# pennneutrinos/chroma

Measured on AMD Instinct MI355X. Metric: photons/sec (propagate_hit), higher is better.
Workload: dtype f32

## Files before the change

chroma_amd/csrc/chroma_hip.hip:

```cpp
#include <math.h>
#include <stdio.h>
#include <stdlib.h>
#include <string.h>
#include <algorithm>

#ifndef CHROMA_EXPERIMENTAL
#define CHROMA_EXPERIMENTAL 0
#endif
#ifndef CHROMA_HYBRID_RENDER
#define CHROMA_HYBRID_RENDER 1
#endif
#include "chroma_internal.h"
#include "propagate_device.h"

#include "kernel_propagate_fused.h"

#include "kernel_step_control.h"

#include "kernels_raycast_crosscheck.h"

#include "kernel_raycast_quad.h"

#include "kernel_raycast_pair.h"

// ... 156 lines not shown
    HIP_TRY(hipMemset(cs.d_counters, 0, sizeof c));
    stats->photon_steps += c.photon_steps;
    stats->nodes_visited += c.nodes_visited;
    stats->triangles_tested += c.triangles_tested;
    stats->stack_overflows += c.stack_overflows;
    stats->stack_spills += c.stack_spills;
    stats->packet_rays += c.packet_rays;
    stats->packet_nodes_visited += c.packet_nodes;
    stats->packet_triangles_tested += c.packet_tris;
    return CHROMA_OK;
}

enum { EV_STEP_BEGIN, EV_PACKET_BEGIN, EV_CAST_BEGIN, EV_CAST_END, EV_PHYSICS_END, EV_STEP_END, EV_PER_STEP };

struct chroma_tracks {
    struct Slab { float4 *rows; uint32_t count; };
    uint64_t nphotons = 0, nrows = 0;
    float4 *rows0 = nullptr;
    uint32_t *offsets = nullptr;
    std::vector<Slab> slabs;
};

static void tracks_release(chroma_ctx *ctx, chroma_tracks *tr)
{
    if (!tr) return;
    for (const chroma_tracks::Slab &s : tr->slabs) chroma_free(ctx, s.rows);
    chroma_free(ctx, tr->rows0);
    chroma_free(ctx, tr->offsets);
    delete tr;
}

namespace { struct PropagateCall; }
static int propagate_order(PropagateCall &call, uint32_t **d_order);

namespace {
struct PropagateCall {
    const CallScope &scope; CallState &cs;
    chroma_ctx *ctx; chroma_geometry *geom;
    CallPlan plan;
    PhotonView pv; chroma_rng rng; chroma_propagate_options opt;
    uint64_t nphotons; uint32_t ncopies;
    uint32_t *in_q, *out_q;
    float4 *work_in, *work_out;
    float4 *rays, *rays_next;
    float4 *final_rec;
    uint32_t final_epoch;
    HitsOut ho;
    bool finalize;
    chroma_propagate_stats acc;
    long long n_upper;
    bool finalized;
    chroma_tracks *tracks;

    hipEvent_t *events(int step) const { return opt.time_kernels ? cs.step_events.data() + EV_PER_STEP * step : nullptr; }

    int load_working()
    {
        const unsigned blocks = (unsigned)std::min<uint64_t>((nphotons + PHYS_BLOCK - 1) / PHYS_BLOCK, (uint64_t)ctx->physics_blocks);
        int rc = scope.clear_words(W_PACKET_USE, W_PACKET_END - W_PACKET_USE); if (rc) return rc;
        uint32_t *d_order = nullptr;
        rc = propagate_order(*this, &d_order); if (rc) return rc;
        hipLaunchKernelGGL(k_load_working, dim3(blocks), dim3(PHYS_BLOCK), 0, ctx->stream, geom->view, pv, in_q, work_in,
                           (uint64_t)nphotons, ncopies, (uint32_t)(nphotons / ncopies), plan.chain ? rays : nullptr,
                           plan.packet == 2 ? cs.d_words + W_PACKET_COHERENT : nullptr, (const uint32_t *)d_order, plan.cast == Cast::LITERAL ? 1 : 0);
        if (d_order) { chroma_free(ctx, d_order); acc.reordered += nphotons; }
#if CHROMA_EXPERIMENTAL
        if (plan.packet)
            hipLaunchKernelGGL(k_packet_decide, dim3(1), dim3(1), 0, ctx->stream, cs.d_words + W_PACKET_COHERENT, cs.d_words + W_PACKET_USE,
                               (uint64_t)nphotons, plan.packet);
#endif
        HIP_TRY(hipGetLastError());
        return CHROMA_OK;
    }

    void launch_step_begin(uint32_t first_n)
    {
        hipLaunchKernelGGL(k_step_begin, dim3(1), dim3(1), 0, ctx->stream, in_q, out_q, cs.d_step,
                           tracks ? 0u : opt.use_weights ? 0xFFFFFFFFu : (uint32_t)(PROP_BLOCK * 16 * 8), first_n);
    }

    void launch_physics(int scatter_first, int fixup)
    {
        StepState *st = cs.d_step;
        float4 *chained = plan.chain ? rays_next : nullptr;
        const bool plain = geom->view.plain_optics != 0;
        bool deal = false;
#if PHYS_DEAL
        deal = plain && !final_rec;
#endif
        const int pb = deal ? PHYS_DEAL_BLOCK : PHYS_BLOCK_OF(!plain);
        unsigned blocks = (unsigned)std::min<long long>((n_upper + pb - 1) / pb, std::max<long long>(1, (long long)ctx->physics_blocks * PHYS_BLOCK / pb));
        if (fixup == 1 && plain) blocks = std::max(std::min(blocks, 64u), blocks / 8);
        DeviceCounters *pc = plan.counting ? cs.d_counters : nullptr;
#if PHYS_DEAL
        if (deal) {
            hipLaunchKernelGGL(k_physics_deal, dim3(blocks), dim3(PHYS_DEAL_BLOCK), 0, ctx->stream, geom->view, pv, st, work_in, out_q, work_out,
                               cs.hit_triangle, cs.hit_distance, rng.seed, rng.photon_id_base, opt.use_weights, scatter_first,
                               cs.retry_list, fixup, pc, chained);
            return;
        }
#endif
        const int literal_rays = fixup == 2 ? 1 : 0;
        with_bool(!plain, [&](auto FULL) {
            hipLaunchKernelGGL((k_physics<FULL>), dim3(blocks), dim3(PHYS_BLOCK_OF(FULL)), 0, ctx->stream, geom->view, pv, st, work_in, out_q,
                               work_out, cs.hit_triangle, cs.hit_distance, rng.seed, rng.photon_id_base, opt.use_weights, scatter_first,
                               cs.retry_list, fixup, pc, chained, final_rec, final_epoch, literal_rays);
        });
    }

    int launch_split_step(int scatter_first, hipEvent_t *ev, uint32_t first_n, bool packet)
    {
        if (n_upper <= 0) return CHROMA_OK;
        StepState *st = cs.d_step;
        const Cast cast = plan.cast;
        const bool exact = cast == Cast::LITERAL || cast == Cast::LITERAL_LANE;
        const dim3 block(PROP_BLOCK);
        auto record = [&](int slot) { return ev ? hipEventRecord(ev[slot], ctx->stream) : hipSuccess; };
        const unsigned rblocks = (unsigned)std::min<long long>((n_upper + PROP_BLOCK - 1) / PROP_BLOCK, 8 * 256);
        auto retry = [&](auto C) {
            hipLaunchKernelGGL((k_raycast_retry<C>), dim3(rblocks), block, 0, ctx->stream, geom->view, rays, st, cs.hit_triangle,
                               cs.hit_distance, cs.retry_list, cs.d_counters);
        };
        launch_step_begin(first_n);
        HIP_TRY(record(EV_STEP_BEGIN));
        if (!plan.chain) {
            unsigned sblocks = (unsigned)std::min<long long>((n_upper + 255) / 256, (long long)ctx->physics_blocks * 4);
            hipLaunchKernelGGL(k_ray_setup, dim3(sblocks), dim3(256), 0, ctx->stream, geom->view, work_in, st, rays,
                               cs.hit_triangle, cs.hit_distance, cs.retry_list, &st->retry, cast == Cast::LITERAL ? 1 : 0);
        }
        HIP_TRY(record(EV_PACKET_BEGIN));
        const uint32_t *skip_quad = nullptr;
#if CHROMA_EXPERIMENTAL
        if (packet) {
            skip_quad = cs.d_words + W_PACKET_USE;
            const unsigned pwaves = (unsigned)std::min<long long>((n_upper + WAVE - 1) / WAVE, (long long)ctx->waves[(int)Cast::QUAD]);
            with_bool(plan.counting, [&](auto C) {
                hipLaunchKernelGGL((k_raycast_packet<C>), dim3(pwaves), block, 0, ctx->stream, geom->view, rays, st, cs.hit_triangle,
                                   cs.hit_distance, cs.retry_list, cs.d_counters, cs.d_words + W_PACKET_USE);
            });
        }
#else
        (void)packet;
#endif
        HIP_TRY(record(EV_CAST_BEGIN));
        const dim3 grid(cast_waves(ctx, cast, n_upper));
        const int chained = plan.chain ? 1 : 0;
        with_bool(plan.counting, [&](auto C) {
            switch (cast) {
            case Cast::PAIR:
                hipLaunchKernelGGL((k_raycast_pair<C>), grid, block, 0, ctx->stream, geom->view, rays, 0, st, cs.hit_triangle,
                                   cs.hit_distance, cs.retry_list, cs.coop_spill, cs.d_counters, ctx->coop_chunk);
                break;
            case Cast::QUAD:
                hipLaunchKernelGGL((k_raycast_quad<C>), grid, block, 0, ctx->stream, geom->view, rays, 0, st, cs.hit_triangle,
                                   cs.hit_distance, cs.retry_list, cs.coop_spill, cs.d_counters, ctx->coop_chunk, chained, skip_quad,
                                   ctx->claim_static);
                break;
            case Cast::COOP:
                hipLaunchKernelGGL((k_raycast_coop<C>), grid, block, 0, ctx->stream, geom->view, rays, 0, st, cs.hit_triangle,
                                   cs.hit_distance, cs.retry_list, cs.coop_spill, cs.d_counters, ctx->coop_chunk);
                break;
            case Cast::WIDE:
                hipLaunchKernelGGL((k_raycast_wide<C>), grid, block, 0, ctx->stream, geom->view, rays, 0, st, cs.hit_triangle,
                                   cs.hit_distance, cs.retry_list, cs.wide_spill, cs.d_counters, ctx->ray_chunk);
                break;
            case Cast::PERSISTENT:
                hipLaunchKernelGGL((k_raycast_persistent<C>), grid, block, 0, ctx->stream, geom->view, rays, 0, st, cs.hit_triangle,
                                   cs.hit_distance, cs.retry_list, cs.d_counters);
                break;
            case Cast::LITERAL:
                hipLaunchKernelGGL((k_raycast_literal<C>), grid, block, 0, ctx->stream, geom->view, rays, st, cs.hit_triangle,
                                   cs.hit_distance, cs.coop_spill, cs.d_counters, ctx->coop_chunk, chained, cs.retry_list,
                                   ctx->claim_static);
                retry(C);
                break;
            case Cast::LITERAL_LANE:
                hipLaunchKernelGGL((k_raycast_retry<C, true>), grid, block, 0, ctx->stream, geom->view, rays, st, cs.hit_triangle,
                                   cs.hit_distance, cs.retry_list, cs.d_counters);
                break;
            }
        });
        HIP_TRY(record(EV_CAST_END));
        launch_physics(scatter_first, exact ? 2 : 0);
        HIP_TRY(record(EV_PHYSICS_END));
        if (!exact) {
            with_bool(plan.counting, retry);
            launch_physics(scatter_first, 1);
        }
        HIP_TRY(record(EV_STEP_END));
        HIP_TRY(hipGetLastError());
        if (plan.chain) std::swap(rays, rays_next);
        return CHROMA_OK;
    }

    int launch_tail(int nsteps, int scatter_first, hipEvent_t *ev, uint32_t first_n, bool *done)
    {
        *done = false;
        const unsigned waves = cast_waves(ctx, Cast::COOP, n_upper);
        if ((long long)waves * 8 < n_upper) return CHROMA_OK;
        launch_step_begin(first_n);
        HitsOut beside; memset(&beside, 0, sizeof beside);
        uint32_t *words = nullptr;
        if (finalize) {
            beside = ho;
            words = cs.d_words;
            int rc = scope.clear_results(); if (rc) return rc;
            if (final_rec)
                hipLaunchKernelGGL(k_mark_tail, dim3(32), dim3(256), 0, ctx->stream, in_q, final_rec, photon_tail_stamp(final_epoch));
            HIP_TRY(hipEventRecord(cs.ev_fork, ctx->stream));
        }
        if (ev) HIP_TRY(hipEventRecord(ev[EV_STEP_BEGIN], ctx->stream));
        with_bool(plan.cast == Cast::LITERAL, [&](auto L) {
            with_bool(plan.counting, [&](auto C) {
                hipLaunchKernelGGL((k_tail_coop<C, L>), dim3(waves), dim3(PROP_BLOCK), 0, ctx->stream, geom->view, pv, cs.d_step, work_in,
                                   rng.seed, rng.photon_id_base, nsteps, opt.use_weights, scatter_first, cs.coop_spill, cs.d_counters, beside, words);
            });
        });
        if (ev) HIP_TRY(hipEventRecord(ev[EV_STEP_END], ctx->stream));
        if (finalize) {
            HIP_TRY(hipStreamWaitEvent(cs.aux_stream, cs.ev_fork, 0));
            launch_finalize(cs.aux_stream, photon_tail_stamp(final_epoch));
            HIP_TRY(hipEventRecord(cs.ev_join, cs.aux_stream));
            HIP_TRY(hipStreamWaitEvent(ctx->stream, cs.ev_join, 0));
            finalized = true;
        }
        HIP_TRY(hipGetLastError());
        *done = true;
        return CHROMA_OK;
    }

    void launch_finalize(hipStream_t stream, uint32_t tail_mark)
    {
        const unsigned blocks = (unsigned)((nphotons + COPY_ITEMS * 256 - 1) / (COPY_ITEMS * 256));
        hipLaunchKernelGGL(k_finalize_hits, dim3(blocks), dim3(256), 0, stream, geom->view, pv, (const float4 *)final_rec, final_epoch,
                           (uint64_t)nphotons, ho, cs.d_words, tail_mark);
    }

    int read_step_times(int steps, int tail_step)
    {
        for (int k = 0; k < steps; k++) {
            const hipEvent_t *ev = events(k);
            float ms = 0.f;
            HIP_TRY(hipEventElapsedTime(&ms, ev[EV_STEP_BEGIN], ev[EV_STEP_END]));
            acc.kernel_ms += ms;
            if (k == tail_step) continue;
            HIP_TRY(hipEventElapsedTime(&ms, ev[EV_CAST_BEGIN], ev[EV_CAST_END]));
            acc.raycast_ms += ms;
            acc.raycast_launches++;
            if (k == 0 && plan.packet) {
                HIP_TRY(hipEventElapsedTime(&ms, ev[EV_PACKET_BEGIN], ev[EV_CAST_BEGIN]));
                acc.packet_ms += ms;
                acc.packet_launches++;
            }
            HIP_TRY(hipEventElapsedTime(&ms, ev[EV_CAST_END], ev[EV_PHYSICS_END]));
            acc.physics_ms += ms;
            acc.physics_launches++;
        }
        return CHROMA_OK;
    }

    int run_device_steps()
    {
        const int max_steps = opt.max_steps;
        HIP_TRY(hipMemsetAsync(cs.d_step, 0, sizeof(StepState), ctx->stream));
        hipLaunchKernelGGL(k_set_word, dim3(1), dim3(1), 0, ctx->stream, in_q, 1u);
        hipLaunchKernelGGL(k_set_word, dim3(1), dim3(1), 0, ctx->stream, out_q, 1u);
        int rc = load_working(); if (rc) return rc;
        const int nev = opt.time_kernels ? EV_PER_STEP * max_steps : 0;
        while ((int)cs.step_events.size() < nev) { hipEvent_t e; HIP_TRY(hipEventCreate(&e)); cs.step_events.push_back(e); }
        const long long few = (long long)PROP_BLOCK * 16 * 8;
        int step = 0, next_check = 1, tail_step = -1;
        bool done = false;
        while (step < max_steps && !done) {
            const int scatter_first = step == 0 ? opt.scatter_first : 0;
            const uint32_t first_n = step == 0 ? (uint32_t)nphotons : 0u;
            if (plan.tail && n_upper < few) {
                rc = launch_tail(max_steps - step, scatter_first, events(step), first_n, &done); if (rc) return rc;
                if (done) { tail_step = step++; break; }
            }
            rc = launch_split_step(scatter_first, events(step), first_n, step == 0 && plan.packet != 0); if (rc) return rc;
            step++;
            std::swap(in_q, out_q);
            std::swap(work_in, work_out);
            if (step == next_check && step < max_steps) {
                rc = scope.read_survivors(in_q, &n_upper); if (rc) return rc;
                if (n_upper <= 0) done = true;
                next_check = (plan.tail_watch && n_upper < 16 * few) ? step + 1 : (step < 8) ? step * 2 : step + 8;
            }
        }
        if (!done) {
            unsigned blocks = (unsigned)std::min<long long>((n_upper + 255) / 256, 4096);
            hipLaunchKernelGGL(k_store_working, dim3(std::max(blocks, 1u)), dim3(256), 0, ctx->stream, geom->view, pv, in_q, work_in);
        }
        HIP_TRY(hipMemcpyAsync(cs.h_step, cs.d_step, sizeof(StepState), hipMemcpyDeviceToHost, ctx->stream));
        HIP_TRY(hipStreamSynchronize(ctx->stream));
        acc.launches += ((const StepState *)cs.h_step)->launches;
        return opt.time_kernels ? read_step_times(step, tail_step) : CHROMA_OK;
    }

    void store_working()
    {
        const unsigned blocks = (unsigned)std::min<long long>((n_upper + 255) / 256, 4096);
        hipLaunchKernelGGL(k_store_working, dim3(std::max(blocks, 1u)), dim3(256), 0, ctx->stream, geom->view, pv, in_q, work_in);
    }

    int run_tracked_steps(uint64_t max_rows)
    {
// ... 83 lines not shown
                HIP_TRY(hipEventElapsedTime(&ms, cs.ev_start, cs.ev_stop));
                acc.kernel_ms += ms;
            }
            step += nsteps;
            scatter_first = 0;
            if (step < max_steps) {
                std::swap(in_q, out_q);
                hipLaunchKernelGGL(k_set_word, dim3(1), dim3(1), 0, ctx->stream, out_q, 1u);
                rc = scope.read_survivors(in_q, &n); if (rc) return rc;
                if (n == 0) break;
            }
        }
        return CHROMA_OK;
    }

    int finish(chroma_hits_request *hr, chroma_propagate_stats *stats, int32_t *aborted)
    {
        int rc = CHROMA_OK;
        if (!finalize) {
            rc = scope.clear_words(W_ABORT); if (rc) return rc;
            const unsigned blocks = (unsigned)std::min<uint64_t>((nphotons + 255) / 256, 4096);
            hipLaunchKernelGGL(k_flags_or, dim3(blocks), dim3(256), 0, ctx->stream, pv.flags, (uint64_t)nphotons, CHROMA_NAN_ABORT,
                               cs.d_words + W_ABORT);
        } else if (!finalized) {
            rc = scope.clear_results(); if (rc) return rc;
            launch_finalize(ctx->stream, 0u);
        }
        HIP_TRY(hipGetLastError());
        rc = scope.read_results(); if (rc) return rc;
        if (hr) hr->nhits = scope.word(W_HIT_COUNT);
        if (aborted) *aborted = (scope.word(W_ABORT) & CHROMA_NAN_ABORT) ? 1 : 0;
        chroma_propagate_stats tmp; memset(&tmp, 0, sizeof tmp);
        chroma_propagate_stats *s = stats ? stats : &tmp;
        rc = stats_read(scope, s); if (rc) return rc;
        if (stats) {
            stats->launches += acc.launches;
            stats->kernel_ms += acc.kernel_ms;
            stats->raycast_ms += acc.raycast_ms;
            stats->raycast_launches += acc.raycast_launches;
            stats->physics_ms += acc.physics_ms;
            stats->physics_launches += acc.physics_launches;
            stats->packet_ms += acc.packet_ms;
            stats->packet_launches += acc.packet_launches;
            stats->reordered += acc.reordered;
        }
        if (s->stack_overflows) return set_error(CHROMA_ERR_STACK, "traversal stack overflowed for %llu rays", (unsigned long long)s->stack_overflows);
        return CHROMA_OK;
    }
};
}

int propagate_settings(const CallScope &scope)
{
    chroma_ctx *ctx = scope.ctx; CallState &cs = scope.state();
    hipDeviceProp_t prop;
    HIP_TRY(hipGetDeviceProperties(&prop, ctx->device));
    ctx->physics_blocks = prop.multiProcessorCount * 8;
    const char *walk = getenv("CHROMA_WALK");
    if (walk) cs.walk = CHROMA_WALK_QUAD;
    for (int w = 0; w < NWALKS; w++) {
        const Walk &row = WALKS[w];
        int per_cu = row.waves_per_cu;
        if (const char *e = getenv(row.waves_env)) per_cu = std::max(1, atoi(e));
        ctx->waves[(int)row.cast] = prop.multiProcessorCount * per_cu;
        if (walk && (!strcmp(walk, row.name) || (row.alias && !strcmp(walk, row.alias)))) cs.walk = w;
    }
#if CHROMA_EXPERIMENTAL
    if (const char *e = getenv("CHROMA_PACKET")) cs.packet_mode = !strcmp(e, "on") ? 1 : !strcmp(e, "auto") ? 2 : 0;
    if (const char *e = getenv("CHROMA_AUTOSORT")) cs.autosort_mode = !strcmp(e, "on") || !strcmp(e, "1") ? 1 : !strcmp(e, "off") || !strcmp(e, "0") ? 0 : 2;
#endif
    if (const char *e = getenv("CHROMA_RAY_CHUNK")) ctx->ray_chunk = std::max(64, atoi(e));
    if (const char *e = getenv("CHROMA_COOP_CHUNK")) ctx->coop_chunk = std::max(8, atoi(e));
    if (const char *e = getenv("CHROMA_CLAIM_STATIC")) { int big = 0, small = 0; if (sscanf(e, "%d:%d", &big, &small) < 2) small = big; ctx->claim_static = std::min(8, std::max(0, big)) | std::min(8, std::max(0, small)) << 4; }
    if (const char *e = getenv("CHROMA_TAIL"))
        cs.tail_mode = !strcmp(e, "fused") ? CHROMA_TAIL_FUSED : !strcmp(e, "split") ? CHROMA_TAIL_SPLIT : CHROMA_TAIL_COOP;
    return CHROMA_OK;
}

extern "C" {

int chroma_propagate_step(chroma_ctx *ctx, chroma_geometry *geom, int32_t first_photon, int32_t nthreads,
                          const uint32_t *d_input_queue, uint32_t *d_output_queue, chroma_rng rng,
                          const chroma_photon_arrays *photons, int32_t max_steps, int32_t use_weights,
                          int32_t scatter_first)
{
    if (!ctx || !geom) return set_error(CHROMA_ERR_INVALID, "bad argument");
    int rc = check_photons(photons, true);
    if (rc) return rc;
    if (first_photon < 0 || nthreads < 0) return set_error(CHROMA_ERR_INVALID, "negative photon range");
    if (nthreads == 0) return CHROMA_OK;
    if ((rc = check_stack(geom))) return rc;
    const CallScope scope(ctx);
    return launch_propagate(scope, scope.state().counting != 0, geom, to_view(photons), rng,
                            {first_photon, nthreads, d_input_queue, d_output_queue, max_steps, use_weights, scatter_first});
}

static int ensure_queues(const CallScope &scope, size_t n)
{
    chroma_ctx *ctx = scope.ctx; CallState &cs = scope.state();
    if (cs.queue_capacity >= n + 1) return CHROMA_OK;
    HIP_TRY(hipStreamSynchronize(ctx->stream));
    const auto buffers = queue_buffers(cs);
    for (const QueueBuffer &b : buffers) { if (*b.ptr) hipFree(*b.ptr); *b.ptr = nullptr; }
    cs.queue_capacity = 0;
    for (const QueueBuffer &b : buffers) HIP_TRY(ctx_malloc(ctx, b.ptr, (n + 1) * b.bytes));
    cs.queue_capacity = n + 1;
    return CHROMA_OK;
}

int chroma_distance_to_mesh(chroma_ctx *ctx, chroma_geometry *geom, int32_t nthreads, const float *d_origin,
                            const float *d_direction, float *d_distance, int32_t *d_triangle)
{
    return chroma_intersect_mesh(ctx, geom, nthreads, d_origin, d_direction, nullptr, d_distance, d_triangle);
}

int chroma_intersect_mesh(chroma_ctx *ctx, chroma_geometry *geom, int32_t nthreads, const float *d_origin,
                          const float *d_direction, const int32_t *d_last_hit, float *d_distance, int32_t *d_triangle)
{
    if (!ctx || !geom || !d_origin || !d_direction || !d_distance) return set_error(CHROMA_ERR_INVALID, "bad argument");
    if (nthreads <= 0) return CHROMA_OK;
    const CallScope scope(ctx);
    return intersect_mesh_in_scope(scope, geom, nthreads, d_origin, d_direction, d_last_hit, d_distance, d_triangle);
}

}

int intersect_mesh_in_scope(const CallScope &scope, chroma_geometry *geom, int32_t nthreads, const float *d_origin, const float *d_direction,
                            const int32_t *d_last_hit, float *d_distance, int32_t *d_triangle)
{
    chroma_ctx *ctx = scope.ctx;
    CallState &cs = scope.state();
    CallPlan plan;
    int rc = check_stack(geom); if (rc) return rc;
    rc = make_plan(cs, geom, -1, -1, -1, &plan); if (rc) return rc;
    if (!plan.isect_quad) {
        const dim3 grid((unsigned)((nthreads + PROP_BLOCK - 1) / PROP_BLOCK)), block(PROP_BLOCK);
        with_bool(plan.counting, [&](auto C) {
            hipLaunchKernelGGL((k_distance_to_mesh<STACK_LDS, C>), grid, block, 0, ctx->stream, geom->view, nthreads, d_origin, d_direction,
                               d_last_hit, d_distance, d_triangle, cs.d_counters);
        });
        HIP_TRY(hipGetLastError());
        return CHROMA_OK;
    }
    HIP_TRY(hipSetDevice(ctx->device));
    rc = ensure_queues(scope, (size_t)nthreads); if (rc) return rc;
    rc = ensure_spill(scope, SPILL_COOP); if (rc) return rc;
    StepState *st = cs.d_step;
    const unsigned blocks = (unsigned)((nthreads + 255) / 256);
    hipLaunchKernelGGL(k_step_set, dim3(1), dim3(1), 0, ctx->stream, st, (uint32_t)nthreads);
    hipLaunchKernelGGL(k_rays_from_arrays, dim3(blocks), dim3(256), 0, ctx->stream, geom->view, (int)nthreads, d_origin, d_direction,
                       d_last_hit, cs.rays, cs.hit_triangle, cs.hit_distance, cs.retry_list, st);
    const unsigned waves = cast_waves(ctx, Cast::QUAD, nthreads);
    with_bool(plan.counting, [&](auto C) {
        hipLaunchKernelGGL((k_raycast_quad<C>), dim3(waves), dim3(PROP_BLOCK), 0, ctx->stream, geom->view, cs.rays, 0, st,
                           cs.hit_triangle, cs.hit_distance, cs.retry_list, cs.coop_spill, cs.d_counters, ctx->coop_chunk, 0, nullptr, ctx->claim_static);
    });
    hipLaunchKernelGGL(k_distance_finish, dim3(blocks), dim3(256), 0, ctx->stream, geom->view, (int)nthreads, cs.rays, cs.hit_triangle,
                       cs.hit_distance, d_distance, d_triangle, cs.retry_list, st);
    with_bool(plan.counting, [&](auto C) {
        hipLaunchKernelGGL((k_distance_retry<C>), dim3(256), dim3(PROP_BLOCK), 0, ctx->stream, geom->view, cs.rays, st,
                           cs.retry_list, d_distance, d_triangle, cs.d_counters);
    });
    HIP_TRY(hipGetLastError());
    return CHROMA_OK;
}

extern "C" {

int chroma_locate_materials(chroma_ctx *ctx, chroma_geometry *geom, int32_t n, const float *d_points, const float direction[3],
                            int32_t outside, int32_t *d_material, int32_t *d_triangle)
{
    if (!ctx || !geom || !d_points || !d_material) return set_error(CHROMA_ERR_INVALID, "bad argument");
    if (n < 0) return set_error(CHROMA_ERR_INVALID, "negative number of points");
    const float dx = direction ? direction[0] : 0.0f, dy = direction ? direction[1] : 0.0f, dz = direction ? direction[2] : 1.0f;
    const float len = sqrtf(dx * dx + dy * dy + dz * dz);
    if (!(len > 0.0f) || !isfinite(len)) return set_error(CHROMA_ERR_INVALID, "probe direction of no length");
    if (n == 0) return CHROMA_OK;
    int rc = check_stack(geom); if (rc) return rc;
    const CallScope scope(ctx);
    CallState &cs = scope.state();
    CallPlan plan;
    rc = make_plan(cs, geom, -1, -1, -1, &plan); if (rc) return rc;
    HIP_TRY(hipSetDevice(ctx->device));
    rc = ensure_queues(scope, (size_t)n); if (rc) return rc;
    int32_t *triangle = d_triangle ? d_triangle : cs.hit_triangle;
    const unsigned blocks = (unsigned)((n + 255) / 256);
    if (!plan.isect_quad) {
        with_bool(plan.counting, [&](auto C) {
            hipLaunchKernelGGL((k_locate_walk<STACK_LDS, C>), dim3((unsigned)((n + PROP_BLOCK - 1) / PROP_BLOCK)), dim3(PROP_BLOCK), 0, ctx->stream,
                               geom->view, (int)n, d_points, dx, dy, dz, triangle, cs.d_counters);
        });
    } else {
        rc = ensure_spill(scope, SPILL_COOP); if (rc) return rc;
        StepState *st = cs.d_step;
        hipLaunchKernelGGL(k_step_set, dim3(1), dim3(1), 0, ctx->stream, st, (uint32_t)n);
        hipLaunchKernelGGL(k_locate_rays, dim3(blocks), dim3(256), 0, ctx->stream, geom->view, (int)n, d_points, dx, dy, dz, cs.rays,
                           cs.hit_triangle, cs.hit_distance, cs.retry_list, st);
        const unsigned waves = cast_waves(ctx, Cast::QUAD, n);
        with_bool(plan.counting, [&](auto C) {
            hipLaunchKernelGGL((k_raycast_quad<C>), dim3(waves), dim3(PROP_BLOCK), 0, ctx->stream, geom->view, cs.rays, 0, st,
                               cs.hit_triangle, cs.hit_distance, cs.retry_list, cs.coop_spill, cs.d_counters, ctx->coop_chunk, 0, nullptr, ctx->claim_static);
        });
        hipLaunchKernelGGL(k_distance_finish, dim3(blocks), dim3(256), 0, ctx->stream, geom->view, (int)n, cs.rays, cs.hit_triangle,
                           cs.hit_distance, cs.hit_distance, triangle, cs.retry_list, st);
        with_bool(plan.counting, [&](auto C) {
            hipLaunchKernelGGL((k_distance_retry<C>), dim3(256), dim3(PROP_BLOCK), 0, ctx->stream, geom->view, cs.rays, st,
                               cs.retry_list, cs.hit_distance, triangle, cs.d_counters);
        });
    }
    hipLaunchKernelGGL(k_locate_material, dim3(blocks), dim3(256), 0, ctx->stream, geom->view, (int)n, triangle, dx, dy, dz, outside, d_material);
    HIP_TRY(hipGetLastError());
    return CHROMA_OK;
}

int chroma_propagate_stats_read(chroma_ctx *ctx, chroma_propagate_stats *stats)
{
    if (!ctx || !stats) return set_error(CHROMA_ERR_INVALID, "bad argument");
    const CallScope scope(ctx);
    return stats_read(scope, stats);
}

int chroma_set_counting(chroma_ctx *ctx, int32_t enabled)
{
    if (!ctx) return set_error(CHROMA_ERR_INVALID, "null ctx");
    CallScope(ctx).state().counting = enabled ? 1 : 0;
    return CHROMA_OK;
}

int chroma_set_walk(chroma_ctx *ctx, int32_t mode)
{
    if (!ctx) return set_error(CHROMA_ERR_INVALID, "null ctx");
    if (mode < 0 || mode >= NWALKS) return set_error(CHROMA_ERR_INVALID, "unknown walk mode %d", mode);
    CallScope(ctx).state().walk = mode;
    return CHROMA_OK;
}

int chroma_set_packet(chroma_ctx *ctx, int32_t mode)
{
    if (!ctx) return set_error(CHROMA_ERR_INVALID, "null ctx");
    if (mode < 0 || mode > 2) return set_error(CHROMA_ERR_INVALID, "unknown packet mode %d", mode);
#if !CHROMA_EXPERIMENTAL
    if (mode != 0) return set_error(CHROMA_ERR_INVALID, "the packet ray cast is an experiment that is not part of this build (csrc/experimental/: build_variants/libchroma_hip_experimental.so)");
#endif
    CallScope(ctx).state().packet_mode = mode;
    return CHROMA_OK;
}

int chroma_set_autosort(chroma_ctx *ctx, int32_t mode)
{
    if (!ctx) return set_error(CHROMA_ERR_INVALID, "null ctx");
    if (mode < 0 || mode > 2) return set_error(CHROMA_ERR_INVALID, "unknown autosort mode %d", mode);
#if !CHROMA_EXPERIMENTAL
    if (mode != 0) return set_error(CHROMA_ERR_INVALID, "the engine-side direction sort is an experiment that is not part of this build (csrc/experimental/: build_variants/libchroma_hip_experimental.so)");
#endif
    CallScope(ctx).state().autosort_mode = mode;
    return CHROMA_OK;
}

int chroma_set_tail(chroma_ctx *ctx, int32_t mode)
{
    if (!ctx) return set_error(CHROMA_ERR_INVALID, "null ctx");
    if (mode != CHROMA_TAIL_COOP && mode != CHROMA_TAIL_SPLIT && mode != CHROMA_TAIL_FUSED)
        return set_error(CHROMA_ERR_INVALID, "unknown tail mode %d", mode);
    CallScope(ctx).state().tail_mode = mode;
    return CHROMA_OK;
}

#if CHROMA_EXPERIMENTAL
#include "experimental/autosort.h"
#else
static int propagate_order(PropagateCall &, uint32_t **d_order) { *d_order = nullptr; return CHROMA_OK; }
#endif

static int ensure_final_records(const CallScope &scope, size_t n)
{
    chroma_ctx *ctx = scope.ctx; CallState &cs = scope.state();
    if (cs.final_capacity >= n) return CHROMA_OK;
    HIP_TRY(hipStreamSynchronize(ctx->stream));
    if (cs.final_rec) hipFree(cs.final_rec);
    cs.final_rec = nullptr; cs.final_capacity = 0;
    HIP_TRY(ctx_malloc(ctx, (void **)&cs.final_rec, n * 4 * sizeof(float4)));
    HIP_TRY(hipMemsetAsync(cs.final_rec, 0, n * 4 * sizeof(float4), ctx->stream));
    cs.final_capacity = n;
    cs.final_epoch = 0;
    return CHROMA_OK;
}

static int propagate_impl(chroma_ctx *ctx, chroma_geometry *geom, const chroma_photon_arrays *photons, uint64_t nphotons,
                          uint32_t ncopies, chroma_rng rng, const chroma_propagate_options &opt,
                          chroma_propagate_stats *stats, int32_t *aborted, chroma_hits_request *hr)
{
    if (!ctx || !geom) return set_error(CHROMA_ERR_INVALID, "bad argument");
    int rc = check_photons(photons, true); if (rc) return rc;
    const CallScope scope(ctx);
    CallState &cs = scope.state();
    CallPlan plan;
    rc = make_plan(cs, geom, opt.walk, opt.tail, opt.counting, &plan); if (rc) return rc;
    if (hr) {
        hr->nhits = 0;
        if (!geom->view.nsolids) return set_error(CHROMA_ERR_INVALID, "geometry has no detector channel map");
        if (hr->dst) { rc = check_photons(hr->dst, false); if (rc) return rc; }
        if ((hr->dst != nullptr) != (hr->d_channels != nullptr)) return set_error(CHROMA_ERR_INVALID, "flat hits need both dst and d_channels");
    }
    if (nphotons >= 0x7fffffffull) return set_error(CHROMA_ERR_INVALID, "at most 2^31-2 photons per call");
    if (ncopies == 0 || nphotons % ncopies) return set_error(CHROMA_ERR_INVALID, "nphotons must be a multiple of ncopies");
    if (aborted) *aborted = 0;
    const bool stepping = opt.max_steps > 0;
    if (nphotons == 0 || (!stepping && !hr)) return CHROMA_OK;
    if (stepping && (rc = check_stack(geom))) return rc;
    HIP_TRY(hipSetDevice(ctx->device));
    if (stepping) {
        rc = ensure_queues(scope, nphotons); if (rc) return rc;
        rc = ensure_spill(scope, plan.spill); if (rc) return rc;
    }
    static const bool records_always = getenv("CHROMA_FINAL_RECORDS") && atoi(getenv("CHROMA_FINAL_RECORDS")) != 0;
    const bool use_records = stepping && (hr != nullptr || records_always) && plan.tail_mode != CHROMA_TAIL_FUSED;
    if (use_records) {
        rc = ensure_final_records(scope, nphotons); if (rc) return rc;
        cs.final_epoch++;
        if (cs.final_epoch == 0u || cs.final_epoch >= 0x7FFFFFFFu) {
            HIP_TRY(hipMemsetAsync(cs.final_rec, 0, cs.final_capacity * 4 * sizeof(float4), ctx->stream));
            cs.final_epoch = 1u;
        }
    }
    PropagateCall call = {scope, cs, ctx, geom, plan, to_view(photons), rng, opt, nphotons, ncopies, cs.queue_a, cs.queue_b, cs.work_a, cs.work_b,
                          cs.rays, cs.rays_b, use_records ? cs.final_rec : nullptr, cs.final_epoch};
    if (hr) {
        call.ho.want = 1;
        call.ho.detection_state = hr->detection_state;
        if (hr->dst) { call.ho.dst = to_view(hr->dst); call.ho.channels = hr->d_channels; call.ho.capacity = hr->capacity; }
        call.ho.hit_count = hr->d_hit_count; call.ho.earliest = hr->d_hit_count ? hr->d_earliest_time_bits : nullptr;
    }
    call.finalize = use_records || hr;
    call.n_upper = (long long)nphotons;
    if (stepping) {
        rc = plan.tail_mode == CHROMA_TAIL_FUSED ? call.run_fused() : call.run_device_steps();
        if (rc) return rc;
    }
    return call.finish(hr, stats, aborted);
}

static chroma_propagate_options default_options(int32_t max_steps, int32_t use_weights, int32_t scatter_first, int32_t time_kernels)
{
    chroma_propagate_options o; memset(&o, 0, sizeof o);
    o.max_steps = max_steps; o.use_weights = use_weights; o.scatter_first = scatter_first; o.time_kernels = time_kernels;
    o.walk = o.tail = o.counting = -1;
    return o;
}

int chroma_propagate(chroma_ctx *ctx, chroma_geometry *geom, const chroma_photon_arrays *photons, uint64_t nphotons,
                     uint32_t ncopies, chroma_rng rng, int32_t max_steps, int32_t use_weights, int32_t scatter_first,
                     int32_t time_kernels, chroma_propagate_stats *stats, int32_t *aborted)
{
// ... 202 lines not shown
```

chroma_amd/csrc/kernel_raycast_quad.h:

```cpp
#pragma once

#ifndef QUAD_PENDING
#define QUAD_PENDING 16
#endif
#ifndef QUAD_STACK
#define QUAD_STACK COOP_STACK
#endif
#define QUAD_OD_WORDS 6
#define QUAD_STRIDE (2 * QUAD_STACK + QUAD_PENDING + QUAD_OD_WORDS + 1)
#ifndef QUAD_REFILL_MIN
#define QUAD_REFILL_MIN 4
#endif
#ifndef QUAD_WAVES_PER_EU
#define QUAD_WAVES_PER_EU 8
#endif
#ifndef QUAD_TIMING
#define QUAD_TIMING 0
#endif
#ifndef QUAD_FLUSH
#define QUAD_FLUSH 8
#endif
#ifndef QUAD_KEEP
#define QUAD_KEEP 7
#endif

template <int QUAD_PERM>
__device__ inline uint32_t quad_xchg(uint32_t v)
{
    return (uint32_t)__builtin_amdgcn_update_dpp((int)v, (int)v, QUAD_PERM, 0xF, 0xF, true);
}
__device__ inline uint32_t quad_min_u32(uint32_t v)
{
    v = min(v, quad_xchg<0xB1>(v));
    v = min(v, quad_xchg<0x4E>(v));
    return v;
}
__device__ inline uint32_t quad_max_u32(uint32_t v)
{
    v = max(v, quad_xchg<0xB1>(v));
    v = max(v, quad_xchg<0x4E>(v));
    asm volatile("" : "+v"(v));
    return v;
}

__device__ inline void box_interval_pk(float ax, float ay, float az, f32x2 bx, f32x2 by, f32x2 bz, uint4 nd, float &tmin, float &tmax)
{
    f32x2 qx = {(float)(nd.x & 0xFFFFu), (float)(nd.x >> 16)};
    f32x2 qy = {(float)(nd.y & 0xFFFFu), (float)(nd.y >> 16)};
    f32x2 qz = {(float)(nd.z & 0xFFFFu), (float)(nd.z >> 16)};
    const f32x2 tx = __builtin_elementwise_fma(qx, (f32x2){ax, ax}, bx);
    const f32x2 ty = __builtin_elementwise_fma(qy, (f32x2){ay, ay}, by);
    const f32x2 tz = __builtin_elementwise_fma(qz, (f32x2){az, az}, bz);
    tmin = __builtin_fmaxf(__builtin_fmaxf(__builtin_fminf(tx.x, tx.y), __builtin_fminf(ty.x, ty.y)),
                           __builtin_fmaxf(__builtin_fminf(tz.x, tz.y), 0.0f));
    tmax = __builtin_fminf(__builtin_fminf(__builtin_fmaxf(tx.x, tx.y), __builtin_fmaxf(ty.x, ty.y)),
                           __builtin_fmaxf(tz.x, tz.y));
}
__device__ inline void box_interval_signed(float ax, float ay, float az, uint32_t sx, uint32_t sy, uint32_t sz,
                                           f32x2 bx, f32x2 by, f32x2 bz, uint4 nd, float &tmin, float &tmax)
{
    const uint32_t x = __builtin_amdgcn_alignbit(nd.x, nd.x, sx), y = __builtin_amdgcn_alignbit(nd.y, nd.y, sy),
                   z = __builtin_amdgcn_alignbit(nd.z, nd.z, sz);
    f32x2 qx = {(float)(x & 0xFFFFu), (float)(x >> 16)};
    f32x2 qy = {(float)(y & 0xFFFFu), (float)(y >> 16)};
    f32x2 qz = {(float)(z & 0xFFFFu), (float)(z >> 16)};
    const f32x2 tx = __builtin_elementwise_fma(qx, (f32x2){ax, ax}, bx);
    const f32x2 ty = __builtin_elementwise_fma(qy, (f32x2){ay, ay}, by);
    const f32x2 tz = __builtin_elementwise_fma(qz, (f32x2){az, az}, bz);
    tmin = __builtin_fmaxf(__builtin_fmaxf(tx.x, ty.x), __builtin_fmaxf(tz.x, 0.0f));
    tmax = __builtin_fminf(__builtin_fminf(tx.y, ty.y), tz.y);
}
__device__ inline uint32_t quad_or_u32(uint32_t v)
{
    v |= quad_xchg<0xB1>(v);
    v |= quad_xchg<0x4E>(v);
    return v;
}

template <bool COUNT>
__global__ __launch_bounds__(PROP_BLOCK) __attribute__((amdgpu_waves_per_eu(QUAD_WAVES_PER_EU, QUAD_WAVES_PER_EU))) void
k_raycast_quad(GeoView g, const float4 *rays, int first_photon, StepState *st,
               int32_t *hit_triangle, float *hit_distance, uint32_t *retry_list, uint2 *spill_base, DeviceCounters *counters,
               int big_chunk, int settle, const uint32_t *skip = nullptr, int static_eighths = 0)
{
    if (skip && *skip != 0u) return;
    const int nthreads = (int)st->n;
    if ((long long)blockIdx.x * 16 >= nthreads) return;
    uint32_t *work_counter = &st->work, *retry_counter = &st->retry;
    const int chunk = ((long long)nthreads > 4ll * big_chunk * (long long)gridDim.x) ? big_chunk : 16;
    WorkClaim wc(nthreads, chunk, static_eighths);
    static_assert(PROP_BLOCK == WAVE, "one wave per workgroup");
    static_assert((QUAD_PENDING & (QUAD_PENDING - 1)) == 0 && QUAD_FLUSH - 1 + 8 <= QUAD_PENDING && QUAD_KEEP < QUAD_FLUSH, "ring of postponed triangles");
    __shared__ uint32_t s_lds[16 * QUAD_STRIDE];
    const unsigned lane = lane_id();
    const unsigned j = lane & 3u, gshift = lane & ~3u, grp = lane >> 2;
    const uint32_t jbit = 1u << (2u * j), below2 = jbit - 1u;
    uint32_t *stack_n = s_lds + grp * QUAD_STRIDE;
    float *stack_t = (float *)(stack_n + QUAD_STACK);
    uint32_t *pending = stack_n + 2 * QUAD_STACK;
    uint2 *spill = spill_base + ((size_t)blockIdx.x * 16 + grp) * COOP_SPILL;
    LaneCounters cnt = {0, 0, 0, 0};

    bool has_ray = false, active = false;
    int slot = 0;
    float *ray_od = (float *)(stack_n + 2 * QUAD_STACK + QUAD_PENDING);
    float rax = 0.f, ray_ = 0.f, raz = 0.f;
    f32x2 rbx = {0.f, 0.f}, rby = {0.f, 0.f}, rbz = {0.f, 0.f};
    uint32_t rsx = 0, rsy = 0, rsz = 0;
    uint32_t last_hit_w = WIDE_NONE;
    int triangle_index = -1;
    uint32_t best_rank = 0;
    float prune_t = cm_inff();
    uint32_t cur = WIDE_NONE;
    int sp = 0, npend = 0;
    uint32_t phead = 0;
    uint32_t loc_next = 0, loc_end = 0;
    bool exhausted = false;
#if QUAD_TIMING
    unsigned long long tq_refill = 0, tq_pop = 0, tq_wait = 0, tq_node = 0, tq_leaf = 0, tq_retire = 0, tq_a, tq_b;
    unsigned tq_iters = 0, tq_rounds = 0, tq_outer = 0, tq_active = 0, tq_tests = 0;
#define TQ_STAMP(v) asm volatile("s_memtime %0\n\ts_waitcnt lgkmcnt(0)" : "=s"(v) :: "memory")
    const unsigned long long tq_start = __builtin_readcyclecounter();
#endif

    for (;;) {
#if QUAD_TIMING
        TQ_STAMP(tq_a); tq_outer++;
#endif
        unsigned long long idle_mask = __ballot(!has_ray && j == 0);
        int n_idle = __popcll(idle_mask);
        bool more = !exhausted || loc_next < loc_end;
        if (more && (n_idle >= QUAD_REFILL_MIN || n_idle == 16)) {
            if (loc_next >= loc_end) {
                const uint32_t base = wc.next(work_counter, lane, exhausted);
                loc_next = min(base, (uint32_t)nthreads);
                loc_end = min(base + (uint32_t)chunk, (uint32_t)nthreads);
            }
            uint32_t idx = loc_next + (uint32_t)__popcll(idle_mask & ((1ull << gshift) - 1ull));
            loc_next = min(loc_end, loc_next + (uint32_t)n_idle);
            if (!has_ray && idx < loc_end) {
                slot = first_photon + (int)idx;
                const float4 *r = rays + 4 * (size_t)slot;
                const float4 r0 = r[0], r1 = r[1];
                if (__float_as_int(r1.w) == 0) {
                    const float4 r2 = r[2], r3 = r[3];
                    if (j == 0) { ray_od[0] = r0.x; ray_od[1] = r1.x; ray_od[2] = r0.y; ray_od[3] = r1.y; ray_od[4] = r0.z; ray_od[5] = r1.z; }
                    { const int lh = __float_as_int(r0.w); last_hit_w = lh >= 0 ? (0x80000000u | (uint32_t)lh) : WIDE_NONE; }
                    rax = r2.x; ray_ = r2.y; raz = r2.z;
                    { const float mx = r2.w * cm_fabsf(rax), my = r2.w * cm_fabsf(ray_), mz = r2.w * cm_fabsf(raz);
                      rbx = (f32x2){r3.x - mx, r3.x + mx}; rby = (f32x2){r3.y - my, r3.y + my}; rbz = (f32x2){r3.z - mz, r3.z + mz}; }
                    rsx = rax < 0.f ? 16u : 0u; rsy = ray_ < 0.f ? 16u : 0u; rsz = raz < 0.f ? 16u : 0u;
                    triangle_index = -1;
                    prune_t = cm_inff();
                    sp = 0;
                    npend = 0;
                    phead = 0;
                    cur = 0;
                    has_ray = true;
                    active = true;
                } else if (settle && j == 0) {
                    const int status = __float_as_int(r1.w);
                    hit_triangle[slot] = status;
                    hit_distance[slot] = 0.0f;
                    if (status == HIT_RETRY) retry_list[atomicAdd(retry_counter, 1u)] = (uint32_t)slot;
                }
            }
        }
        if (!__any(has_ray)) {
            if (exhausted && loc_next >= loc_end) break;
            continue;
        }

#if QUAD_TIMING
        TQ_STAMP(tq_b); tq_refill += tq_b - tq_a;
#endif
        more = !exhausted || loc_next < loc_end;
        const int stop_at = more ? max(0, (int)__popcll(__ballot(active) & 0x1111111111111111ull) - (int)QUAD_REFILL_MIN) : 0;
        do {
#if QUAD_TIMING
            TQ_STAMP(tq_a); tq_iters++; tq_active += (unsigned)__popcll(__ballot(active && j == 0));
#endif
            __builtin_amdgcn_s_setprio(3);
            if (__any(sp > QUAD_STACK)) {
                while (active && cur == WIDE_NONE && sp > QUAD_STACK) {
                    sp--;
                    const uint2 se = spill[sp - QUAD_STACK];
                    cur = (__uint_as_float(se.y) > prune_t) ? WIDE_NONE : se.x;
                }
            }
            while (active && cur == WIDE_NONE) {
                if (sp == 0) { active = false; break; }
                sp--;
                const uint32_t n = stack_n[sp];
                const float t = stack_t[sp];
                cur = (t > prune_t) ? WIDE_NONE : n;
            }
#if QUAD_TIMING
            TQ_STAMP(tq_b); tq_pop += tq_b - tq_a;
#endif
            if (active) {
                const uint4 *np = g.wnodes + 8 * (size_t)cur + 2 * j;
                const uint4 ea = np[0], eb = np[1];
#if QUAD_TIMING
                asm volatile("s_waitcnt vmcnt(0)" ::: "memory");
                TQ_STAMP(tq_a); tq_wait += tq_a - tq_b;
#endif
                __builtin_amdgcn_s_setprio(0);
                if (COUNT && j == 0) cnt.nodes += 8;
                float ta, tb, fa, fb;
                box_interval_signed(rax, ray_, raz, rsx, rsy, rsz, rbx, rby, rbz, ea, ta, fa);
                box_interval_signed(rax, ray_, raz, rsx, rsy, rsz, rbx, rby, rbz, eb, tb, fb);
                const bool pa = !(ta > fa) & !(ta > prune_t);
                const bool pb = !(tb > fb) & !(tb > prune_t);
                const bool fa_leaf = __builtin_amdgcn_inverse_ballot_w64(__builtin_amdgcn_sicmp((int)ea.w, 0, 40)),
                           fb_leaf = __builtin_amdgcn_inverse_ballot_w64(__builtin_amdgcn_sicmp((int)eb.w, 0, 40));
                const bool la = pa & fa_leaf, lb = pb & fb_leaf;
                const bool ia = pa & !fa_leaf, ib = pb & !fb_leaf;
                const uint32_t qm = quad_or_u32((((ib ? 2u * jbit : 0u) | (ia ? jbit : 0u)) << 8) | (lb ? 2u * jbit : 0u) | (la ? jbit : 0u));
                {
                    const uint32_t sa = (phead + (uint32_t)npend + __popc(__builtin_amdgcn_ubfe(qm, 0u, 2u * j))) & (QUAD_PENDING - 1u);
                    if (la) pending[sa] = ea.w;
                    if (lb) pending[(sa + (la ? 1u : 0u)) & (QUAD_PENDING - 1u)] = eb.w;
                    npend += __popc(qm & 0xFFu);
                }
                cur = WIDE_NONE;
                const uint32_t mi = qm >> 8;
                if (mi) {
                    const uint32_t ka = ia ? ((__float_as_uint(ta) & ~7u) | (2u * j)) : 0xFFFFFFFFu;
                    const uint32_t kb = ib ? ((__float_as_uint(tb) & ~7u) | (2u * j + 1u)) : 0xFFFFFFFFu;
                    const uint32_t ne = quad_min_u32(min(ka, kb)) & 7u;
                    const bool ea_near = __builtin_amdgcn_inverse_ballot_w64(__builtin_amdgcn_uicmp(ne, 2u * j, 32)),
                               eb_near = __builtin_amdgcn_inverse_ballot_w64(__builtin_amdgcn_uicmp(ne, 2u * j + 1u, 32));
                    const bool na = ia & ea_near, nb = ib & eb_near;
                    cur = quad_max_u32(na ? ea.w : (nb ? eb.w : 0u));
                    const bool qa = ia && !na, qb = ib && !nb;
                    const uint32_t mo = mi & ~(1u << ne);
                    int pos = sp + __popc(mo & below2);
                    sp += __popc(mo);
                    if (!__any(sp > QUAD_STACK)) {
                        if (qa) { stack_n[pos] = ea.w; stack_t[pos] = ta; pos++; }
                        if (qb) { stack_n[pos] = eb.w; stack_t[pos] = tb; }
                    } else
                    {
                        if (qa) {
                            if (pos < QUAD_STACK) { stack_n[pos] = ea.w; stack_t[pos] = ta; }
                            else if (pos < QUAD_STACK + COOP_SPILL) { spill[pos - QUAD_STACK] = make_uint2(ea.w, __float_as_uint(ta)); if (COUNT) atomicAdd(&counters->stack_spills, 1ull); }
                            pos++;
                        }
                        if (qb) {
                            if (pos < QUAD_STACK) { stack_n[pos] = eb.w; stack_t[pos] = tb; }
                            else if (pos < QUAD_STACK + COOP_SPILL) { spill[pos - QUAD_STACK] = make_uint2(eb.w, __float_as_uint(tb)); if (COUNT) atomicAdd(&counters->stack_spills, 1ull); }
                        }
                        if (sp > QUAD_STACK + COOP_SPILL) { atomicAdd(&counters->stack_overflows, 1ull); sp = QUAD_STACK + COOP_SPILL; }
                    }
                }
            }
#if QUAD_TIMING
            TQ_STAMP(tq_b); tq_node += tq_b - tq_a;
#endif
        } while (!__any(npend >= QUAD_FLUSH) && (int)__popcll(__ballot(active) & 0x1111111111111111ull) > stop_at);
        __builtin_amdgcn_wave_barrier();
#if QUAD_TIMING
        TQ_STAMP(tq_a);
#endif

        if (__any(npend > (active ? QUAD_KEEP : 0))) do {
#if QUAD_TIMING
            tq_rounds++; tq_tests += (unsigned)__popcll(__ballot(npend > 0 && (int)j < min(npend, 4)));
#endif
            {
                const int take = min(npend, 4);
                bool hit = false;
                float distance = 0.0f;
                uint32_t tri_w = 0, rank = 0xFFFFFFFFu;
                if ((int)j < take) tri_w = pending[(phead + j) & (QUAD_PENDING - 1u)];
                const uint32_t tri = tri_w & 0x7FFFFFFFu;
                if ((int)j < take && tri_w != last_hit_w) {
                    if (COUNT) cnt.tris++;
                    hit = intersect_triangle_edges((f32x2){ray_od[0], ray_od[1]}, (f32x2){ray_od[2], ray_od[3]}, (f32x2){ray_od[4], ray_od[5]},
                                                   g.tri_isect + 3 * (size_t)tri, distance, rank);
                }
                const uint32_t dkey = hit ? __float_as_uint(distance) : 0x7F800000u;
                const uint32_t dmin = quad_min_u32(dkey);
                const float dm = __uint_as_float(dmin);
                const bool cand = hit && dkey == dmin;
                const uint32_t rm = quad_min_u32(cand ? rank : 0xFFFFFFFFu);
                const uint32_t wtri = quad_max_u32((cand && rank == rm) ? tri + 1u : 0u) - 1u;
                const bool better = dmin != 0x7F800000u && (dm < prune_t || (dm == prune_t && rm < best_rank));
                triangle_index = better ? (int)wtri : triangle_index;
                prune_t = better ? dm : prune_t;
                best_rank = better ? rm : best_rank;
                phead = (phead + (uint32_t)take) & (QUAD_PENDING - 1u);
                npend -= take;
            }
        } while (__any(npend > (active ? QUAD_KEEP : 0)));


#if QUAD_TIMING
        TQ_STAMP(tq_b); tq_leaf += tq_b - tq_a;
#endif
        if (has_ray && !active) {
            if (j == 0) {
                hit_triangle[slot] = triangle_index;
                hit_distance[slot] = triangle_index == -1 ? -1.0f : prune_t;
                if (triangle_index == HIT_RETRY) retry_list[atomicAdd(retry_counter, 1u)] = (uint32_t)slot;
            }
            has_ray = false;
        }
    }

#if QUAD_TIMING
    if (lane == 0 && (blockIdx.x & 1023u) == 0u && nthreads > 1000000) {
        const unsigned long long total = __builtin_readcyclecounter() - tq_start;
        printf("QT rays %d wave %u total %llu refill %llu pop %llu wait %llu node %llu leaf %llu outer %u iters %u active %u rounds %u tests %u\n",
               nthreads, blockIdx.x, total, tq_refill, tq_pop, tq_wait, tq_node, tq_leaf, tq_outer, tq_iters, tq_active, tq_rounds, tq_tests);
    }
#endif
    flush_counters<COUNT>(cnt, counters, lane);
}
```

Before: 904.2 million.

## Prefetch next ray records into LDS via global_load_lds during quad raycast

After each refill, the quad raycast kernel issues asynchronous global-to-LDS loads of the next up-to-8 ray records, so later refills can read them from shared memory instead of waiting on global loads. The refill now loads all four rows unconditionally and computes idle rank with mbcnt, counting lanes with j==3. It adds dynamic LDS per workgroup (512 bytes) at all three launch sites, plus a vmcnt(0) wait before staged reads. This risks lower occupancy, and the ballot change may cause subtle rank mismatches.

```diff
diff --git a/chroma_amd/csrc/chroma_hip.hip b/chroma_amd/csrc/chroma_hip.hip
--- a/chroma_amd/csrc/chroma_hip.hip
+++ b/chroma_amd/csrc/chroma_hip.hip
@@ -332,7 +332,7 @@
                                    cs.hit_distance, cs.retry_list, cs.coop_spill, cs.d_counters, ctx->coop_chunk);
                 break;
             case Cast::QUAD:
-                hipLaunchKernelGGL((k_raycast_quad<C>), grid, block, 0, ctx->stream, geom->view, rays, 0, st, cs.hit_triangle,
+                hipLaunchKernelGGL((k_raycast_quad<C>), grid, block, QUAD_STAGE_BYTES, ctx->stream, geom->view, rays, 0, st, cs.hit_triangle,
                                    cs.hit_distance, cs.retry_list, cs.coop_spill, cs.d_counters, ctx->coop_chunk, chained, skip_quad,
                                    ctx->claim_static);
                 break;
@@ -722,7 +722,7 @@
                        d_last_hit, cs.rays, cs.hit_triangle, cs.hit_distance, cs.retry_list, st);
     const unsigned waves = cast_waves(ctx, Cast::QUAD, nthreads);
     with_bool(plan.counting, [&](auto C) {
-        hipLaunchKernelGGL((k_raycast_quad<C>), dim3(waves), dim3(PROP_BLOCK), 0, ctx->stream, geom->view, cs.rays, 0, st,
+        hipLaunchKernelGGL((k_raycast_quad<C>), dim3(waves), dim3(PROP_BLOCK), QUAD_STAGE_BYTES, ctx->stream, geom->view, cs.rays, 0, st,
                            cs.hit_triangle, cs.hit_distance, cs.retry_list, cs.coop_spill, cs.d_counters, ctx->coop_chunk, 0, nullptr, ctx->claim_static);
     });
     hipLaunchKernelGGL(k_distance_finish, dim3(blocks), dim3(256), 0, ctx->stream, geom->view, (int)nthreads, cs.rays, cs.hit_triangle,
@@ -768,7 +768,7 @@
                            cs.hit_triangle, cs.hit_distance, cs.retry_list, st);
         const unsigned waves = cast_waves(ctx, Cast::QUAD, n);
         with_bool(plan.counting, [&](auto C) {
-            hipLaunchKernelGGL((k_raycast_quad<C>), dim3(waves), dim3(PROP_BLOCK), 0, ctx->stream, geom->view, cs.rays, 0, st,
+            hipLaunchKernelGGL((k_raycast_quad<C>), dim3(waves), dim3(PROP_BLOCK), QUAD_STAGE_BYTES, ctx->stream, geom->view, cs.rays, 0, st,
                                cs.hit_triangle, cs.hit_distance, cs.retry_list, cs.coop_spill, cs.d_counters, ctx->coop_chunk, 0, nullptr, ctx->claim_static);
         });
         hipLaunchKernelGGL(k_distance_finish, dim3(blocks), dim3(256), 0, ctx->stream, geom->view, (int)n, cs.rays, cs.hit_triangle,
diff --git a/chroma_amd/csrc/kernel_raycast_quad.h b/chroma_amd/csrc/kernel_raycast_quad.h
--- a/chroma_amd/csrc/kernel_raycast_quad.h
+++ b/chroma_amd/csrc/kernel_raycast_quad.h
@@ -20,6 +20,16 @@
 #ifndef QUAD_FLUSH
 #define QUAD_FLUSH 8
 #endif
+#ifndef QUAD_REFILL_ROWS4
+#define QUAD_REFILL_ROWS4 1
+#endif
+#ifndef QUAD_STAGE
+#define QUAD_STAGE 8
+#endif
+#if QUAD_STAGE && !QUAD_REFILL_ROWS4
+#error "the staged records are read by the four-row refill"
+#endif
+#define QUAD_STAGE_BYTES (QUAD_STAGE * 64)
 #ifndef QUAD_KEEP
 #define QUAD_KEEP 7
 #endif
@@ -92,8 +102,12 @@
     static_assert(PROP_BLOCK == WAVE, "one wave per workgroup");
     static_assert((QUAD_PENDING & (QUAD_PENDING - 1)) == 0 && QUAD_FLUSH - 1 + 8 <= QUAD_PENDING && QUAD_KEEP < QUAD_FLUSH, "ring of postponed triangles");
     __shared__ uint32_t s_lds[16 * QUAD_STRIDE];
+#if QUAD_STAGE
+    extern __shared__ float4 s_stage[];
+    uint32_t n_staged = 0;
+#endif
     const unsigned lane = lane_id();
-    const unsigned j = lane & 3u, gshift = lane & ~3u, grp = lane >> 2;
+    const unsigned j = lane & 3u, grp = lane >> 2;
     const uint32_t jbit = 1u << (2u * j), below2 = jbit - 1u;
     uint32_t *stack_n = s_lds + grp * QUAD_STRIDE;
     float *stack_t = (float *)(stack_n + QUAD_STACK);
@@ -117,8 +131,8 @@
     uint32_t loc_next = 0, loc_end = 0;
     bool exhausted = false;
 #if QUAD_TIMING
-    unsigned long long tq_refill = 0, tq_pop = 0, tq_wait = 0, tq_node = 0, tq_leaf = 0, tq_retire = 0, tq_a, tq_b;
-    unsigned tq_iters = 0, tq_rounds = 0, tq_outer = 0, tq_active = 0, tq_tests = 0;
+    unsigned long long tq_refill = 0, tq_pop = 0, tq_wait = 0, tq_node = 0, tq_leaf = 0, tq_retire = 0, tq_drain = 0, tq_a, tq_b;
+    unsigned tq_iters = 0, tq_rounds = 0, tq_outer = 0, tq_active = 0, tq_tests = 0, tq_refills = 0, tq_taken = 0;
 #define TQ_STAMP(v) asm volatile("s_memtime %0\n\ts_waitcnt lgkmcnt(0)" : "=s"(v) :: "memory")
     const unsigned long long tq_start = __builtin_readcyclecounter();
 #endif
@@ -127,23 +141,52 @@
 #if QUAD_TIMING
         TQ_STAMP(tq_a); tq_outer++;
 #endif
-        unsigned long long idle_mask = __ballot(!has_ray && j == 0);
+        unsigned long long idle_mask = __ballot(!has_ray && j == 3);
         int n_idle = __popcll(idle_mask);
         bool more = !exhausted || loc_next < loc_end;
         if (more && (n_idle >= QUAD_REFILL_MIN || n_idle == 16)) {
+#if QUAD_TIMING
+            asm volatile("s_waitcnt vmcnt(0)" ::: "memory");
+            TQ_STAMP(tq_b); tq_drain += tq_b - tq_a;
+#endif
             if (loc_next >= loc_end) {
                 const uint32_t base = wc.next(work_counter, lane, exhausted);
                 loc_next = min(base, (uint32_t)nthreads);
                 loc_end = min(base + (uint32_t)chunk, (uint32_t)nthreads);
-            }
-            uint32_t idx = loc_next + (uint32_t)__popcll(idle_mask & ((1ull << gshift) - 1ull));
+#if QUAD_STAGE
+                n_staged = 0;
+#endif
+            }
+            const uint32_t rank = __builtin_amdgcn_mbcnt_hi((uint32_t)(idle_mask >> 32), __builtin_amdgcn_mbcnt_lo((uint32_t)idle_mask, 0u));
+            uint32_t idx = loc_next + rank;
             loc_next = min(loc_end, loc_next + (uint32_t)n_idle);
+#if QUAD_TIMING
+            tq_refills++; tq_taken += (unsigned)__popcll(__ballot(!has_ray && j == 0 && idx < loc_end));
+#endif
             if (!has_ray && idx < loc_end) {
                 slot = first_photon + (int)idx;
                 const float4 *r = rays + 4 * (size_t)slot;
+#if QUAD_REFILL_ROWS4
+                float4 r0, r1, r2, r3;
+#if QUAD_STAGE
+                if (rank < n_staged) {
+                    asm volatile("s_waitcnt vmcnt(0)" ::: "memory");
+                    uint32_t stage_at = (uint32_t)(size_t)(__attribute__((address_space(3))) float4 *)s_stage;
+                    asm volatile("" : "+s"(stage_at));
+                    typedef float f32x4 __attribute__((ext_vector_type(4)));
+                    const volatile __attribute__((address_space(3))) f32x4 *sr = (const volatile __attribute__((address_space(3))) f32x4 *)(size_t)(stage_at + 64u * rank);
+                    const f32x4 q0 = sr[0], q1 = sr[1], q2 = sr[2], q3 = sr[3];
+                    r0 = make_float4(q0.x, q0.y, q0.z, q0.w); r1 = make_float4(q1.x, q1.y, q1.z, q1.w);
+                    r2 = make_float4(q2.x, q2.y, q2.z, q2.w); r3 = make_float4(q3.x, q3.y, q3.z, q3.w);
+                } else
+#endif
+                { r0 = r[0]; r1 = r[1]; r2 = r[2]; r3 = r[3]; }
+                if (__float_as_int(r1.w) == 0) {
+#else
                 const float4 r0 = r[0], r1 = r[1];
                 if (__float_as_int(r1.w) == 0) {
                     const float4 r2 = r[2], r3 = r[3];
+#endif
                     if (j == 0) { ray_od[0] = r0.x; ray_od[1] = r1.x; ray_od[2] = r0.y; ray_od[3] = r1.y; ray_od[4] = r0.z; ray_od[5] = r1.z; }
                     { const int lh = __float_as_int(r0.w); last_hit_w = lh >= 0 ? (0x80000000u | (uint32_t)lh) : WIDE_NONE; }
                     rax = r2.x; ray_ = r2.y; raz = r2.z;
@@ -165,6 +208,15 @@
                     if (status == HIT_RETRY) retry_list[atomicAdd(retry_counter, 1u)] = (uint32_t)slot;
                 }
             }
+#if QUAD_STAGE
+            n_staged = min((uint32_t)QUAD_STAGE, loc_end - loc_next);
+            uint32_t row;
+            asm volatile("v_mbcnt_lo_u32_b32 %0, -1, 0\n\tv_mbcnt_hi_u32_b32 %0, -1, %0" : "=v"(row));
+            if (row < 4u * n_staged) {
+                __builtin_amdgcn_global_load_lds((const __attribute__((address_space(1))) float4 *)(rays + 4 * ((size_t)first_photon + loc_next) + row),
+                                                 (__attribute__((address_space(3))) float4 *)s_stage, 16, 0, 0);
+            }
+#endif
         }
         if (!__any(has_ray)) {
             if (exhausted && loc_next >= loc_end) break;
@@ -312,8 +364,8 @@
 #if QUAD_TIMING
     if (lane == 0 && (blockIdx.x & 1023u) == 0u && nthreads > 1000000) {
         const unsigned long long total = __builtin_readcyclecounter() - tq_start;
-        printf("QT rays %d wave %u total %llu refill %llu pop %llu wait %llu node %llu leaf %llu outer %u iters %u active %u rounds %u tests %u\n",
-               nthreads, blockIdx.x, total, tq_refill, tq_pop, tq_wait, tq_node, tq_leaf, tq_outer, tq_iters, tq_active, tq_rounds, tq_tests);
+        printf("QT rays %d wave %u total %llu refill %llu pop %llu wait %llu node %llu leaf %llu outer %u iters %u active %u rounds %u tests %u refills %u taken %u drain %llu\n",
+               nthreads, blockIdx.x, total, tq_refill, tq_pop, tq_wait, tq_node, tq_leaf, tq_outer, tq_iters, tq_active, tq_rounds, tq_tests, tq_refills, tq_taken, tq_drain);
     }
 #endif
     flush_counters<COUNT>(cnt, counters, lane);
```

Result: no change. 912.1 million, median of 6 (+0.9%).
